# Ignaciagothe/tda-eeg-audio

Measured on AMD Instinct MI355X. Metric: windows/sec end-to-end (dist->Rips H0/H1->Wasserstein), 47-ch EEG, higher is better.
Workload: dtype f64; 1 GPU; configs[4]+configs[2]: 1416 recordings x 5 bands x 15 selected windows = 106200 (EEG 47x250 f64, audio 250 f64) window pairs per pass, the whole job; per pair corr->dist->Rips H0/H1 (EEG 47 pts), tau per recording-band, Takens dim 3 sub 2 + Rips (audio, 23..123 pts over the bands), Wasserstein H0+H1, features, per-recording reductions; one all-gather of the (1416, 5x48) rows per pass; windows_per_pass=106200, windows_per_gpu_per_pass=106200, input_bytes_per_gpu=10195200000, batches_per_pass=1, windows_per_batch=106200, parallelism=recordings dealt over 1 rank(s), one all-gather per pass, batches_in_flight=3, hip_graph=True, batches_rerun_with_full_ladder=0

## Files before the change

### tda_eeg_audio_amd/csrc/rips.hip

```cpp
#include "common.h"
#include "corr_dist_dev.h"
#include <stdlib.h>

#ifndef CLOUD_NB
#define CLOUD_NB 8192
#endif
#ifndef NARROW_NT
#define NARROW_NT 512
#endif
#ifndef NARROW_WAVES
#define NARROW_WAVES 6
#endif
#if defined(TDA_PROFILE) && !defined(TDA_PROFILE_STOPS_ONLY)
#define NARROW_NB (NARROW_NT == 384 ? 1536 : 1024)
#else
#define NARROW_NB (NARROW_NT == 384 ? 1536 : 2048)
#endif
#define NARROW_EMAX 7626
#define NT_MAX 512
#define RANK_NONE 0x7fffu

#ifdef TDA_PROFILE
__device__ unsigned long long g_prof[48];
#ifdef TDA_PROFILE_STOPS_ONLY
// ... 16 lines not shown
        prof_t0 = prof_t1;                                                 \
    } while (0)
#define PROF_COUNT(i, v) do { if (threadIdx.x == 0) prof_lds[i] += (unsigned long long)(v); } while (0)
#define PROF_FLUSH()                                                       \
    do {                                                                   \
        __syncthreads();                                                   \
        if (threadIdx.x < 48 && prof_lds[threadIdx.x]) atomicAdd(&g_prof[threadIdx.x], prof_lds[threadIdx.x]); \
    } while (0)
#endif
__device__ int g_stop_after;
extern "C" __attribute__((visibility("default"))) int tda_profile_stop_after(int n)
{
    return hipMemcpyToSymbol(HIP_SYMBOL(g_stop_after), &n, sizeof(int)) != hipSuccess;
}
#define PROF_STOP(n, cleanup) do { if (g_stop_after == (n)) { cleanup; return; } } while (0)
#define PROF_STOPC(n, cleanup) do { if (g_stop_after == (n) + 100 * prof_chunk) { cleanup; return; } } while (0)
extern "C" __attribute__((visibility("default"))) int tda_profile_read(unsigned long long* out, int reset)
{
    if (hipMemcpyFromSymbol(out, HIP_SYMBOL(g_prof), sizeof(unsigned long long) * 48) != hipSuccess) return 1;
    if (reset) {
        unsigned long long z[48] = {0};
        if (hipMemcpyToSymbol(HIP_SYMBOL(g_prof), z, sizeof(z)) != hipSuccess) return 1;
    }
    return 0;
}
#else
#define PROF_BEGIN() do {} while (0)
#define PROF_RESUME() do {} while (0)
#define PROF_MARK(i) do {} while (0)
#define PROF_COUNT(i, v) do {} while (0)
#define PROF_FLUSH() do {} while (0)
#define PROF_STOP(n, cleanup) do {} while (0)
#define PROF_STOPC(n, cleanup) do {} while (0)
#endif

#define LDS_ORDER() asm volatile("" ::: "memory")

#define LAUNDER(v) asm volatile("" : "+v"(v))
#define WAVE_SYNC()                                            \
    do {                                                       \
        __builtin_amdgcn_fence(__ATOMIC_ACQ_REL, "workgroup"); \
        __builtin_amdgcn_wave_barrier();                       \
    } while (0)

struct SweepShared {
    u64 alive[8];
    int cov_min[2], status, spare, k1, nk, more;
};

typedef unsigned short pk_u16 __attribute__((ext_vector_type(2)));
typedef short pk_i16 __attribute__((ext_vector_type(2)));

template <int W, typename WT>
struct __attribute__((aligned(sizeof(WT)))) Psi {
    WT w[W];
};
template <int W, typename WT>
__device__ __forceinline__ Psi<W, WT> pxor(Psi<W, WT> a, Psi<W, WT> b)
{
    Psi<W, WT> r;
#pragma unroll
    for (int i = 0; i < W; ++i) r.w[i] = a.w[i] ^ b.w[i];
    return r;
}
template <int W, typename WT>
__device__ __forceinline__ bool pnz(Psi<W, WT> a)
{
    WT o = 0;
#pragma unroll
    for (int i = 0; i < W; ++i) o |= a.w[i];
    return o != 0;
}
template <int W, typename WT>
__device__ __forceinline__ Psi<W, WT> pzero()
{
    Psi<W, WT> r;
#pragma unroll
    for (int i = 0; i < W; ++i) r.w[i] = 0;
    return r;
}

__device__ __forceinline__ double wave_min_f64(double v)
{
#pragma unroll
    for (int off = 32; off > 0; off >>= 1) { const double o = __shfl_xor(v, off, 64); v = o < v ? o : v; }
    return v;
}
__device__ __forceinline__ double wave_max_f64(double v)
{
#pragma unroll
    for (int off = 32; off > 0; off >>= 1) { const double o = __shfl_xor(v, off, 64); v = o > v ? o : v; }
    return v;
}

__device__ __forceinline__ int tri2(int v) { return (v * (v - 1)) >> 1; }
__device__ __forceinline__ int pair_index(int x, int y) { return x > y ? tri2(x) + y : tri2(y) + x; }

__device__ __forceinline__ int edge_row(int e)
{
    const int a = (int)((1.0f + __builtin_amdgcn_sqrtf(1.0f + 8.0f * (float)e)) * 0.5f);
    const int t = tri2(a);
    return a + (t + a <= e ? 1 : 0) - (t > e ? 1 : 0);
}

#ifndef TDA_NO_EDGE_TABLE
struct EdgeTable {
    u16 v[8192 + 512];
    constexpr EdgeTable() : v()
    {
        int a = 1, b = 0;
        for (int e = 0; e < 8192 + 512; ++e) { v[e] = (u16)((a << 8) | b); if (++b == a) { ++a; b = 0; } }
    }
};
__device__ const EdgeTable g_edge_ab = EdgeTable();
__device__ __forceinline__ u32 edge_ab(int e) { return (u32)g_edge_ab.v[e]; }
#else
__device__ __forceinline__ u32 edge_ab(int e) { const int a = edge_row(e); return (u32)((a << 8) | (e - tri2(a))); }
#endif

struct WgVote {
    u32* slots;
    int parity;
};
template <int NT>
__device__ __forceinline__ bool wg_any(WgVote& v, bool p)
{
    static_assert(NT % 64 == 0 && NT <= 512, "slots are read as one or two 16-byte words; slots beyond NT / 64 hold zero");
    const bool w = __ballot(p) != 0ull;
    u32* s = v.slots + 8 * v.parity;
    if ((threadIdx.x & 63) == 0) s[threadIdx.x >> 6] = w ? 1u : 0u;
    __syncthreads();
    v.parity ^= 1;
    const uint4 x = *reinterpret_cast<const uint4*>(s);
    u32 r = x.x | x.y | x.z | x.w;
    if (NT > 256) { const uint4 y = *reinterpret_cast<const uint4*>(s + 4); r |= y.x | y.y | y.z | y.w; }
    return r != 0u;
}
template <int NT>
__device__ __forceinline__ bool wg_all(WgVote& v, bool p) { return !wg_any<NT>(v, !p); }

__device__ __forceinline__ int wave_incl_scan_i32(int v)
{
#define TDA_DPP_ADD_(CTRL, RM) v += __builtin_amdgcn_update_dpp(0, v, CTRL, RM, 0xF, true)
    TDA_DPP_ADD_(0x111, 0xF);
    TDA_DPP_ADD_(0x112, 0xF);
    TDA_DPP_ADD_(0x114, 0xF);
    TDA_DPP_ADD_(0x118, 0xF);
    TDA_DPP_ADD_(0x142, 0xA);
    TDA_DPP_ADD_(0x143, 0xC);
#undef TDA_DPP_ADD_
    return v;
}

__device__ __forceinline__ int edge_flat(u32 pk) { return tri2((int)(pk >> 8)) + (int)(pk & 255u); }

struct Bucketer {
    float dmin, scale, top;
    __device__ __forceinline__ int operator()(u32 key) const
    {
        const float x = fminf((sortable_f32(key) - dmin) * scale, top);
        const int b = (int)x;
        return b < 0 ? 0 : b;
    }
};

template <int NT>
__device__ __forceinline__ void effective_threshold(int n, u32 tkey, const u32* vmax, u32 kmin_thread, u32* red, u32& teff_out, u32& kmin_out)
{
    const int tid = threadIdx.x;
    const int lane = tid & 63;
    const u32 m0 = lane < n ? vmax[lane] : 0xffffffffu, m1 = lane + 64 < n ? vmax[lane + 64] : 0xffffffffu;
    const u32 renc = wave_min_u32_dpp(m0 < m1 ? m0 : m1);
    teff_out = renc < tkey ? renc : tkey;
    if (tid == 0) red[1] = 0xffffffffu;
    __syncthreads();
    const u32 kmin = wave_min_u32_dpp(kmin_thread);
    if (lane == 63) atomicMin(&red[1], kmin);
    __syncthreads();
    kmin_out = red[1];
}

template <int NT, int NB, bool WANT_KEYS>
__device__ __forceinline__ int rank_edges(const u32* key32, int E, u32 teff, u32 kmin, u16* members, u32* cursor, int* wsum, u16* rank,
                          u16* ord, u32* skey)
{
    static_assert(NB % (2 * NT) == 0, "every thread scans whole words");
    constexpr int WPT = NB / NT / 2;
    const int tid = threadIdx.x, lane = tid & 63, wave = tid >> 6;
    Bucketer bk;
    bk.dmin = sortable_f32(kmin);
    bk.top = (float)(NB - 1);
    bk.scale = bk.top / (sortable_f32(teff) - bk.dmin);
    for (int i = tid; i < NB / 2; i += NT) cursor[i] = 0u;
    __syncthreads();
#pragma unroll 4
    for (int e = tid; e < E; e += NT) {
        const u32 k = key32[e];
        u32 b = 0xffffu;
        if (k <= teff) { b = (u32)bk(k); atomicAdd(&cursor[b >> 1], 1u << (16 * (b & 1))); }
        rank[e] = (u16)b;
    }
    __syncthreads();
    {
        u32 w[WPT];
        int s = 0;
#pragma unroll
        for (int i = 0; i < WPT; ++i) {
            const u32 x = cursor[tid * WPT + i];
            const int c0 = (int)(x & 0xffffu), c1 = (int)(x >> 16);
            w[i] = (u32)s | ((u32)(s + c0) << 16);
            s += c0 + c1;
        }
        const int incl = wave_incl_scan_i32(s);
        if (lane == 63) wsum[wave] = incl;
        __syncthreads();
        int basep = incl - s;
        for (int q = 0; q < wave; ++q) basep += wsum[q];
        const u32 add = (u32)basep * 0x00010001u;
#pragma unroll
        for (int i = 0; i < WPT; ++i) cursor[tid * WPT + i] = w[i] + add;
    }
    __syncthreads();
#pragma unroll 4
    for (int e = tid; e < E; e += NT) {
        const u32 b = rank[e];
        if (b != 0xffffu) {
            const int sh = 16 * (int)(b & 1u);
            const u32 old = atomicAdd(&cursor[b >> 1], 1u << sh);
            members[(old >> sh) & 0xffffu] = (u16)e;
        }
    }
    __syncthreads();
    const u16* cur16 = reinterpret_cast<const u16*>(cursor);
    const int Ev = uni((int)cur16[NB - 1]);
#pragma unroll 4
    for (int e = tid; e < E; e += NT) {
        const u32 b = rank[e];
        u32 r = RANK_NONE;
        if (b != 0xffffu) {
            const u32 k = key32[e];
            const int lo = b ? (int)cur16[b - 1] : 0, hi = (int)cur16[b];
            int c = 0;
            for (int j = lo; j < hi; ++j) {
                const u32 m = members[j];
                const u32 km = key32[m];
                c += (km < k || (km == k && m < (u32)e)) ? 1 : 0;
            }
            r = (u32)(lo + c);
        }
        rank[e] = (u16)r;
    }
    __syncthreads();
#pragma unroll 4
    for (int e = tid; e < E; e += NT) {
        const u32 r = rank[e];
        if (r != RANK_NONE) {
            ord[r] = (u16)edge_ab(e);
            if (WANT_KEYS) skey[r] = key32[e];
        }
    }
    __syncthreads();
    return Ev;
}

#if defined(TDA_PROFILE) && !defined(TDA_PROFILE_STOPS_ONLY)
#define NARROW_LDS ((160 * 1024 / 3 / 1280) * 1280 - 384)
#else
#define NARROW_LDS ((160 * 1024 / 3 / 1280) * 1280)
#endif
#define NARROW_PMAX 124
#define NARROW_DIM 3
#ifdef TDA_DEBUG_PTS
#define NL_GUARD 16
#else
#define NL_GUARD 0
#endif
#define NL_A16(x) (((x) + 15) & ~15)
struct NL {
    static constexpr int E = NARROW_EMAX;
    static constexpr int RANK = 0;
    static constexpr int PSI = NL_A16(2 * E) + NL_GUARD;
    static constexpr int MEMBERS = NL_A16(4 * E);
    static constexpr int CURSOR = NL_A16(MEMBERS + 2 * E);
    static constexpr int RSCR = CURSOR + 2 * NARROW_NB;
    static constexpr int TOTAL = NARROW_LDS;
    static constexpr int AUX = TOTAL - NL_GUARD - NL_A16(NARROW_PMAX * NARROW_DIM * 8);
    static constexpr int MISC = AUX - NL_GUARD - NL_A16(8752 + 8 * 32);
    static constexpr int REGION = MISC - NL_GUARD - PSI;
    static_assert(RSCR + 720 <= AUX - NL_GUARD, "the ranking arrays must end in front of the points");
    static_assert(MEMBERS >= 4 * (E + 1) && CURSOR >= MEMBERS + 2 * (E + 3), "room for the walk's padding (rank_edges_narrow)");
    static_assert(REGION >= 2 * E + 8 * 512, "the first chunks must fit: class vectors of 2 NT ranks next to the whole of ord");
};

template <int NT, int NB>
__device__ __forceinline__ int rank_edges_narrow(const u32* key32, int E, u32 teff, u32 kmin, u16* members, u32* cursor, int* wsum,
                                                 u16* rank, u16* ord)
{
    static_assert(NB % (2 * NT) == 0, "every thread scans whole words");
    static_assert(NB <= 0x8000, "bucket indices are parked in 16 bits, 0xffff = beyond the threshold");
    constexpr int WPT = NB / NT / 2;
    constexpr int EPT = 2 * ((NARROW_EMAX + 2 * NT - 1) / (2 * NT));
    const int tid = threadIdx.x, lane = tid & 63, wave = tid >> 6;
    Bucketer bk;
    bk.dmin = sortable_f32(kmin);
    bk.top = (float)(NB - 1);
    bk.scale = bk.top / (sortable_f32(teff) - bk.dmin);
// ... 23 lines not shown
        }
        const int incl = wave_incl_scan_i32(s);
        if (lane == 63) wsum[wave] = incl;
        __syncthreads();
        int basep = incl - s;
        for (int q = 0; q < wave; ++q) basep += wsum[q];
        const u32 add = (u32)basep * 0x00010001u;
#pragma unroll
        for (int i = 0; i < WPT; ++i) cursor[tid * WPT + i] = w[i] + add;
        if (tid == NT - 1) {
            const int total = basep + s;
            members[total] = (u16)NARROW_EMAX; members[total + 1] = (u16)NARROW_EMAX; members[total + 2] = (u16)NARROW_EMAX;
            const_cast<u32*>(key32)[NARROW_EMAX] = 0xffffffffu;
        }
    }
    __syncthreads();
#pragma unroll
    for (int i = 0; i < EPT; ++i) {
        const u32 b = i & 1 ? rk[i >> 1] >> 16 : rk[i >> 1] & 0xffffu;
        if (b != 0xffffu) {
            const int sh = 16 * (int)(b & 1u);
            const u32 old = atomicAdd(&cursor[b >> 1], 1u << sh);
            members[(old >> sh) & 0xffffu] = (u16)(tid + i * NT);
        }
    }
    __syncthreads();
    const u16* cur16 = reinterpret_cast<const u16*>(cursor);
    const int Ev = uni((int)cur16[NB - 1]);
#pragma unroll
    for (int i = 0; i < EPT; ++i) {
        const u32 e = (u32)(tid + i * NT);
        const u32 b = i & 1 ? rk[i >> 1] >> 16 : rk[i >> 1] & 0xffffu;
        u32 r = RANK_NONE;
        if (b != 0xffffu) {
            const u32 k = key32[e];
            const u64 me = ((u64)k << 32) | e;
            const int lo = b ? (int)cur16[b - 1] : 0, hi = (int)cur16[b];
            int c = 0;
            for (int j = lo; j < hi; j += 4) {
                u32 m[4], km[4];
#pragma unroll
                for (int t = 0; t < 4; ++t) m[t] = (u32)members[j + t];
#pragma unroll
                for (int t = 0; t < 4; ++t) km[t] = key32[m[t]];
#pragma unroll
                for (int t = 0; t < 4; ++t) c += ((((u64)km[t] << 32) | m[t]) < me) ? 1 : 0;
            }
            r = (u32)(lo + c);
        }
        if (i & 1) rk[i >> 1] = (rk[i >> 1] & 0xffffu) | (r << 16); else rk[i >> 1] = (rk[i >> 1] & 0xffff0000u) | r;
    }
    __syncthreads();
#pragma unroll
    for (int i = 0; i < EPT; ++i) {
        const int e = tid + i * NT;
        if (e < E) {
            const u32 r = i & 1 ? rk[i >> 1] >> 16 : rk[i >> 1] & 0xffffu;
            rank[e] = (u16)r;
            if (r != RANK_NONE) ord[r] = (u16)edge_ab(e);
        }
    }
    __syncthreads();
    return Ev;
}

struct RipsOut {
    double* h0; int h0_cap; int* h0_cnt;
    double* h1; int h1_cap; int* h1_cnt;
    int* status;
    int* retry_list = nullptr;
};

struct RipsLayout {
    int off_members;
    int off_rank, off_ord, off_aux, off_misc;
    int total;
    int off_psi, psi_bytes, off_cursor, off_rscr;
    int guard[5], n_guard;
};

#define TDA_WIN_LDS_GUARD 0x100
#ifndef TDA_SOLO_PRIO
#define TDA_SOLO_PRIO 3
#endif
#define TDA_SOLO_BEGIN() __builtin_amdgcn_s_setprio(TDA_SOLO_PRIO)
#define TDA_SOLO_END() __builtin_amdgcn_s_setprio(0)

#define TDA_POLL_LIMIT (1 << 16)
#ifndef TDA_TURN_SLEEP
#define TDA_TURN_SLEEP 4
#endif
#ifdef TDA_DEBUG_PTS
__device__ int g_fault;
extern "C" __attribute__((visibility("default"))) int tda_debug_inject(int what)
{
    return hipMemcpyToSymbol(HIP_SYMBOL(g_fault), &what, sizeof(int)) != hipSuccess;
}
#define TDA_FAULT(n) (g_fault == (n))
#else
#define TDA_FAULT(n) false
#endif
#ifdef TDA_DEBUG_PTS
#define GUARD_BYTES 16
__device__ __forceinline__ void guard_write(unsigned char* smem, const RipsLayout& L)
{
    if ((int)threadIdx.x < 4 * L.n_guard) reinterpret_cast<u32*>(smem + L.guard[threadIdx.x >> 2] - GUARD_BYTES)[threadIdx.x & 3] = 0xC0FFEE00u + threadIdx.x;
    __syncthreads();
}
__device__ __forceinline__ int guard_check(unsigned char* smem, const RipsLayout& L)
{
    __syncthreads();
    bool bad = false;
    if ((int)threadIdx.x < 4 * L.n_guard) bad = reinterpret_cast<u32*>(smem + L.guard[threadIdx.x >> 2] - GUARD_BYTES)[threadIdx.x & 3] != 0xC0FFEE00u + threadIdx.x;
    return __syncthreads_or(bad ? 1 : 0) ? TDA_WIN_LDS_GUARD : 0;
}
#else
#define GUARD_BYTES 0
__device__ __forceinline__ void guard_write(unsigned char*, const RipsLayout&) {}
__device__ __forceinline__ int guard_check(unsigned char*, const RipsLayout&) { return 0; }
#endif

#define MISC_COMP 0
#define MISC_CAND 512
#define MISC_WV (512 + 128)
#define MISC_MIN (512 + 192)
#define MISC_DONE (512 + 208)
#define MISC_SORTCNT (512 + 224)
#define MISC_SHARED (MISC_DONE + NT_MAX)
#define MISC_CKEY (MISC_SHARED + 96)
#define MISC_LIST MISC_CKEY
#define MISC_LIST_BYTES (4 * NT_MAX + 1280)
#define MISC_ADJ (MISC_LIST + MISC_LIST_BYTES)
#define MISC_ADJC (MISC_ADJ + 128 * 16)
#define MISC_BRANK (MISC_ADJC + 128 * 16)
#define MISC_BYTES(ncls) (MISC_BRANK + 8 * (ncls))

template <int NT, int NVW, int W, typename WT, bool NARROW, class KEYFN>
__device__ __forceinline__ void rips_sweep(int n, int E, int Ev, const u16* rank, const u16* ord, Psi<W, WT>* psi, int psi_bytes,
                           unsigned char* misc, KEYFN keyfn, double* h0, int h0_cap, double* h1, int h1_cap,
                           int& out_k0, int& out_k1, int& out_status)
{
    static_assert(!NARROW || W == 1, "the narrow layout is the point-cloud first pass");
    int psi_cap = 0;
    const int tid0 = threadIdx.x;
    const int lane0 = tid0 & 63, wave = uni(tid0 >> 6);
    int* brank = reinterpret_cast<int*>(misc + MISC_BRANK);
    u64* cand = reinterpret_cast<u64*>(misc + MISC_CAND);
    unsigned char* done = misc + MISC_DONE;
    SweepShared* shared = reinterpret_cast<SweepShared*>(misc + MISC_SHARED);
    u64* adj = reinterpret_cast<u64*>(misc + MISC_ADJ);
    constexpr int WB = 8 * (int)sizeof(WT);
    float* bkey = reinterpret_cast<float*>(misc + MISC_BRANK + 4 * WB * W);
    u64* adjc = reinterpret_cast<u64*>(misc + MISC_ADJC);

    if constexpr (!NARROW) for (int e = tid0; e < E; e += NT) psi[e] = pzero<W, WT>();
    for (int i = tid0; i < WB * W; i += NT) { brank[i] = -1; bkey[i] = 0.f; }
    for (int i = tid0; i < 256; i += NT) { adj[i] = 0ull; adjc[i] = 0ull; }
    if (tid0 == 0) {
        u32* lc = reinterpret_cast<u32*>(misc + MISC_MIN);
        lc[0] = 0u; lc[1] = 0xffffffffu; lc[2] = 0u;
        lc[3] = 0u;
        shared->status = 0;
    }
    if (tid0 < 16) {
        reinterpret_cast<u32*>(misc + MISC_WV)[tid0] = 0u;
        cand[tid0] = 0ull;
    }
    __syncthreads();

    WgVote vote{reinterpret_cast<u32*>(misc + MISC_WV), 0};
    WT alive[W];
#pragma unroll
    for (int c = 0; c < W; ++c) alive[c] = 0;
    int k0 = 0, k1 = 0, merges = 0, status = 0;
    int compA = lane0, compB = lane0 + 64;

    int clen = NT;
    int ordcls = 0;
    int cov_next = tid0;
#ifdef TDA_PROFILE
    int prof_rneed = 0, prof_chunk = -1;
#endif
    PROF_RESUME();
    for (int r0 = 0; r0 < Ev && !status; r0 += clen) {
        int tid = tid0;
        LAUNDER(tid);
        const int lane = tid & 63;
        clen = NT;
        PROF_MARK(15);
#ifdef TDA_PROFILE
        ++prof_chunk;
#endif
        PROF_COUNT(23, 1);
        const int r = r0 + tid;
        const bool valid = r < Ev;
        int a = 1, b = 0;
        if (valid) { const u32 pk = ord[r]; a = (int)(pk >> 8); b = (int)(pk & 255u); }
        const int tab = tri2(a) + b;
        const int slot = NARROW ? r : tab;
        if constexpr (NARROW) {
            psi_cap = (psi_bytes - 2 * (E - r0)) >> 2;
            if (r < psi_cap) psi[r] = pzero<W, WT>();
        }
        u64 M[NVW], M0[NVW];
        u64 Aj[NVW], Bj[NVW];
#pragma unroll
        for (int w = 0; w < NVW; ++w) { M[w] = 0; M0[w] = 0; Aj[w] = 0; Bj[w] = 0; }
        if (valid) {
#pragma unroll
            for (int w = 0; w < NVW; ++w) { Aj[w] = adj[2 * a + w]; Bj[w] = adj[2 * b + w]; M0[w] = Aj[w] & Bj[w]; }
        }
        {
            volatile u32* turn = reinterpret_cast<volatile u32*>(misc + MISC_MIN) + 2;
            if (wave > 0) {
                int trips = 0;
                for (;;) {
                    const u32 t = (u32)uni((int)*turn);
                    if (t >= (u32)wave) break;
                    if (++trips > TDA_POLL_LIMIT) { if (lane == 0) turn[1] = 1u; break; }
                    if (t + 1u < (u32)wave) __builtin_amdgcn_s_sleep(TDA_TURN_SLEEP); else __builtin_amdgcn_s_sleep(0);
                }
            }
            __builtin_amdgcn_fence(__ATOMIC_ACQUIRE, "workgroup");
            if (valid) {
#pragma unroll
                for (int w = 0; w < NVW; ++w) M[w] = (Aj[w] | adjc[2 * a + w]) & (Bj[w] | adjc[2 * b + w]);
                atomicOr(reinterpret_cast<unsigned long long*>(&adjc[2 * a + (b >> 6)]), 1ull << (b & 63));
                atomicOr(reinterpret_cast<unsigned long long*>(&adjc[2 * b + (a >> 6)]), 1ull << (a & 63));
            }
            LDS_ORDER();
            if (lane == 0 && !(TDA_FAULT(1) && wave == 3)) *turn = (u32)wave + 1u;
        }
        if (valid) {
            const int ta0 = tri2(a), tb0 = tri2(b);
#pragma unroll
            for (int w = 0; w < NVW; ++w) {
                u64 cc = (Aj[w] | adjc[2 * a + w]) & (Bj[w] | adjc[2 * b + w]) & ~M[w];
                while (cc) {
                    const int v0 = 64 * w + __builtin_ctzll(cc); cc &= cc - 1ull;
                    const bool ok1 = cc != 0ull; const int v1 = ok1 ? 64 * w + __builtin_ctzll(cc) : v0; cc &= cc - 1ull;
                    const int t0 = tri2(v0), t1 = tri2(v1);
                    const u32 xa0 = rank[v0 < a ? ta0 + v0 : t0 + a], xb0 = rank[v0 < b ? tb0 + v0 : t0 + b];
                    const u32 xa1 = rank[v1 < a ? ta0 + v1 : t1 + a], xb1 = rank[v1 < b ? tb0 + v1 : t1 + b];
                    if ((int)(xa0 > xb0 ? xa0 : xb0) < r) M[w] |= 1ull << (v0 & 63);
                    if (ok1 && (int)(xa1 > xb1 ? xa1 : xb1) < r) M[w] |= 1ull << (v1 & 63);
                }
            }
        }
        u64 many = 0;
#pragma unroll
        for (int w = 0; w < NVW; ++w) many |= M[w];
        const bool is_cand = valid && many == 0;
        int vstar = 0, d1 = 0, d2 = 0, q1 = 0, q2 = 0;
        {
            u64 many0 = 0;
#pragma unroll
            for (int w = 0; w < NVW; ++w) many0 |= M0[w];
            if (many0) {
                if (NVW == 1 || M0[0]) vstar = __builtin_ctzll(M0[0]);
                else vstar = 64 + __builtin_ctzll(M0[NVW - 1]);
            } else if (many) {
                if (NVW == 1 || M[0]) vstar = __builtin_ctzll(M[0]);
                else vstar = 64 + __builtin_ctzll(M[NVW - 1]);
            }
            if (valid && many != 0) {
                d1 = pair_index(a, vstar); d2 = pair_index(b, vstar);
                q1 = (int)rank[d1] - r0; q2 = (int)rank[d2] - r0;
                if (TDA_FAULT(2) && tid == 77 && q1 >= 0) q1 = tid;
            }
        }
        PROF_MARK(4);
        PROF_STOPC(11, out_k0 = k0; out_k1 = k1; out_status = 0);
        u64* mbal = reinterpret_cast<u64*>(misc + MISC_COMP);
        u64* zbal = mbal + 8;
        int* offs = reinterpret_cast<int*>(mbal + 16);
        u16* freebits = reinterpret_cast<u16*>(misc + MISC_CKEY);
        float mykey = 0.f;
        if (is_cand) mykey = keyfn(r, a, b);
        {
            const u64 bal = __ballot(is_cand), zb = __ballot(is_cand && mykey == 0.0f);
            if (lane == 0) { cand[wave] = bal; zbal[wave] = zb; }
        }
        done[tid] = 0;
        __syncthreads();
        PROF_MARK(21);
        PROF_STOPC(12, out_k0 = k0; out_k1 = k1; out_status = 0);
        int nfree = 0;
#pragma unroll
        for (int c = 0; c < W; ++c) nfree += __builtin_popcountll((u64)(WT)~alive[c]);
        int ncand = 0;
#pragma unroll
        for (int w = 0; w < NT / 64; ++w) ncand += __builtin_popcountll(cand[w]);
        int btot = 0;
        if (ncand > 0) {
        const bool par = ncand > 24;
        const int lblA0 = compA, lblB0 = compB;
        int qpar = NT;
        if (par) {
            int* bcomp = reinterpret_cast<int*>(misc + MISC_LIST + 1024);
            u32* bbest2 = reinterpret_cast<u32*>(bcomp + 128);
            int* bpar = reinterpret_cast<int*>(bcomp + 384);
            auto rounds = [&](int limit) {
                if (wave == 0) { bcomp[lane] = lblA0; bcomp[64 + lane] = lblB0; }
                if (tid < 256) bbest2[tid] = 0xffffffffu;
                __syncthreads();
                bool live = is_cand && tid < limit, picked = false;
                for (int round = 0; round < 64; ++round) {
                    u32* bbest = bbest2 + 128 * (round & 1);
                    int ca = 0, cb2 = 0;
                    if (live) {
                        ca = bcomp[a]; cb2 = bcomp[b];
                        if (ca == cb2) live = false;
                        else { atomicMin(&bbest[ca], (u32)tid); atomicMin(&bbest[cb2], (u32)tid); }
                    }
                    if (!wg_any<NT>(vote, live)) break;
                    if (live && (bbest[ca] == (u32)tid || bbest[cb2] == (u32)tid)) { picked = true; live = false; }
                    if (wave == 0) {
                        TDA_SOLO_BEGIN();
                        int pp[2];
#pragma unroll
                        for (int h = 0; h < 2; ++h) {
                            const int me = lane + 64 * h;
                            pp[h] = me;
                            const u32 bp = bbest[me];
                            if (bp != 0xffffffffu) {
                                const u32 pk = ord[r0 + (int)bp];
                                const int oa = bcomp[pk >> 8], ob = bcomp[pk & 255u];
                                pp[h] = oa == me ? ob : oa;
                                if (bbest[pp[h]] == bp && me < pp[h]) pp[h] = me;
                            }
                        }
                        bpar[lane] = pp[0]; bpar[64 + lane] = pp[1];
                        for (int it = 0; it < 8; ++it) {
                            const int p0 = bpar[lane], p1 = bpar[64 + lane];
                            const int g0 = bpar[p0], g1 = bpar[p1];
                            if (__ballot(g0 != p0 || g1 != p1) == 0ull) break;
                            bpar[lane] = g0; bpar[64 + lane] = g1;
                        }
                        const int c0 = bcomp[lane], c1 = bcomp[64 + lane];
                        const int n0 = bpar[c0], n1 = bpar[c1];
                        bcomp[lane] = n0; bcomp[64 + lane] = n1;
                        u32* other = bbest2 + 128 * ((round + 1) & 1);
                        other[lane] = 0xffffffffu; other[64 + lane] = 0xffffffffu;
                        TDA_SOLO_END();
                    }
                    __syncthreads();
                }
                const u64 mb = __ballot(picked);
                if (lane == 0) mbal[wave] = mb;
                __syncthreads();
            };
            rounds(NT);
            int nbirth = 0, wcut = -1, before = 0;
#pragma unroll
            for (int w = 0; w < NT / 64; ++w) {
                const int nb = __builtin_popcountll(cand[w] & ~mbal[w]);
                if (wcut < 0 && nbirth + nb > nfree) { wcut = w; before = nbirth; }
                nbirth += nb;
            }
            if (wcut >= 0) {
                u64 bw = cand[wcut] & ~mbal[wcut];
                for (int k = before; k < nfree; ++k) bw &= bw - 1ull;
                qpar = 64 * wcut + __builtin_ctzll(bw);
                PROF_COUNT(26, 1);
                __syncthreads();
                rounds(qpar);
            }
            if (wave == 0) { compA = bcomp[lane]; compB = bcomp[64 + lane]; }
        }
        if (wave == 0) {
            TDA_SOLO_BEGIN();
            const u64 candv = cand[lane & 7];
            int q = par ? qpar : NT, births = 0;
            const bool walk = !par;
            for (int g = 0; g < NT / 64 && walk; ++g) {
                u64 cb = q == NT ? rl64(candv, g) : 0ull;
                u64 mm = 0ull;
                if (cb) {
                    PROF_COUNT(20, __builtin_popcountll(cb));
                    const u32 pkv = ord[r0 + 64 * g + lane < E ? r0 + 64 * g + lane : E - 1];
                    while (cb) {
                        const int l = __builtin_ctzll(cb);
                        cb &= cb - 1;
                        const u32 pk = rl32(pkv, l);
                        const int qa = (int)(pk >> 8), qb = (int)(pk & 255u);
                        int ca, cbb;
                        if (NVW == 1) {
                            ca = (int)rl32((u32)compA, qa);
                            cbb = (int)rl32((u32)compA, qb);
                        } else {
                            const int a0 = (int)rl32((u32)compA, qa & 63), a1 = (int)rl32((u32)compB, qa & 63);
                            const int b0 = (int)rl32((u32)compA, qb & 63), b1 = (int)rl32((u32)compB, qb & 63);
                            ca = qa < 64 ? a0 : a1;
                            cbb = qb < 64 ? b0 : b1;
                        }
                        const bool same = ca == cbb, open = q == NT;
                        q = (open && same && births == nfree) ? 64 * g + l : q;
                        births += same ? 1 : 0;
                        const int cnew = (q == NT) ? ca : cbb;
                        compA = compA == cbb ? cnew : compA;
                        if (NVW == 2) compB = compB == cbb ? cnew : compB;
                        mm |= (!same && q == NT) ? (1ull << l) : 0ull;
                    }
                }
                if (lane == 0) mbal[g] = mm;
            }
            int nb = 0, nr = 0, nm = 0;
            if (lane < NT / 64) {
                u64 cg = cand[lane];
                if (64 * lane >= q) cg = 0ull;
                else if (q < 64 * lane + 64) cg &= (1ull << (q - 64 * lane)) - 1ull;
                const u64 mg = mbal[lane], zg = zbal[lane];
                nb = __builtin_popcountll(cg & ~mg); nr = __builtin_popcountll(mg & ~zg); nm = __builtin_popcountll(mg);
            }
            int pb = 0, pr = 0, tb = 0, tr = 0, tm = 0;
#pragma unroll
            for (int w = 0; w < NT / 64; ++w) {
                const int xb = (int)rl32((u32)nb, w), xr = (int)rl32((u32)nr, w), xm = (int)rl32((u32)nm, w);
                if (w < lane) { pb += xb; pr += xr; }
                tb += xb; tr += xr; tm += xm;
            }
            if (lane < NT / 64) { offs[lane] = pb; offs[8 + lane] = pr; }
            if (lane == 0) { offs[16] = tb; offs[17] = tr; offs[18] = tm; offs[19] = q; }
            TDA_SOLO_END();
        } else {
            for (int t = tid - 64; t < WB * W; t += NT - 64) {
                const int cw = t / WB, bit = t & (WB - 1);
                int rk = 0;
                bool fr = false;
#pragma unroll
                for (int c = 0; c < W; ++c) {
                    const WT f_ = (WT)~alive[c];
                    if (c < cw) rk += __builtin_popcountll((u64)f_);
                    if (c == cw) { rk += __builtin_popcountll((u64)(f_ & (((WT)1 << bit) - (WT)1))); fr = (f_ >> bit) & (WT)1; }
                }
                if (fr) freebits[rk] = (u16)t;
// ... 17 lines not shown
            if (row) {
                const int pos = k0 + rpre;
                if (pos < h0_cap) { h0[2 * pos] = 0.0; h0[2 * pos + 1] = (double)mykey; }
            }
            k0 += rtot; merges += mtot;
            if (birth) {
                const int idx = (int)freebits[bpre];
                const int cw = idx / WB, bit = idx & (WB - 1);
                Psi<W, WT> nv = pzero<W, WT>();
#pragma unroll
                for (int c = 0; c < W; ++c)
                    if (c == cw) nv.w[c] = ((WT)1 << bit);
                if (!NARROW || r < psi_cap) psi[slot] = nv;
                brank[idx] = r;
                bkey[idx] = mykey;
            }
            if (W == 1 && wave == 0 && btot > 0) {
                const int nal = __builtin_popcountll((u64)alive[0]);
                if (lane >= nal && lane < nal + btot) ordcls = (int)freebits[lane - nal];
            }
            int left = btot;
#pragma unroll
            for (int c = 0; c < W; ++c) {
                const u64 f_ = (u64)(WT)~alive[c];
                const int pc = __builtin_popcountll(f_);
                if (left >= pc) { alive[c] = (WT)~(WT)0; left -= pc; }
                else if (left > 0) {
                    int lo = 0, hi = 63;
                    while (lo < hi) {
                        const int mid = (lo + hi) >> 1;
                        if (__builtin_popcountll(f_ & ((2ull << mid) - 1ull)) >= left) hi = mid; else lo = mid + 1;
                    }
                    alive[c] |= (WT)(f_ & ((2ull << lo) - 1ull));
                    left = 0;
                }
            }
        }
        }
        if (status) break;
        PROF_MARK(5);
        PROF_STOPC(14, out_k0 = k0; out_k1 = k1; out_status = 0);
        bool quiet = btot == 0;
#pragma unroll
        for (int c = 0; c < W; ++c) quiet = quiet && alive[c] == 0;
        u32* lcnt = reinterpret_cast<u32*>(misc + MISC_MIN);
        if (quiet) PROF_COUNT(24, 1);
#ifdef TDA_PROFILE
        if (!quiet) prof_rneed = r0 + clen;
#endif
        if constexpr (NARROW) {
            if (!quiet && r0 + NT > psi_cap) { status |= TDA_WIN_CLASS_OVERFLOW; break; }
        }
        if (!quiet) {
        const bool apparent = valid && many != 0 && tid < clen;
        bool pending = apparent;
        Psi<W, WT> base = pzero<W, WT>();
        const int s1 = NARROW ? q1 + r0 : d1, s2 = NARROW ? q2 + r0 : d2;
        if (apparent && q1 < 0 && q2 < 0) {
            base = pxor(psi[s1], psi[s2]);
            psi[slot] = base;
            pending = false;
        }
        volatile unsigned char* vdone = done;
        LDS_ORDER();
        if (!pending) vdone[tid] = 1;
#ifdef TDA_PROFILE
#ifndef TDA_PROFILE_STOPS_ONLY
        if (pending) atomicAdd(&prof_lds[33], 1ull);
#endif
        PROF_COUNT(34, 1);
#endif
        int idle_trips = 0;
        while (__ballot(pending)) {
            PROF_COUNT(32, 1);
            bool ready = false;
            if (pending) ready = (q1 < 0 || vdone[q1]) && (q2 < 0 || vdone[q2]);
            const u64 rbal = __ballot(ready);
            __builtin_amdgcn_fence(__ATOMIC_ACQUIRE, "workgroup");
            if (ready) {
                base = pxor(psi[s1], psi[s2]);
                psi[slot] = base;
                LDS_ORDER();
                vdone[tid] = 1;
                pending = false;
            }
            if (!rbal) {
                if (++idle_trips > TDA_POLL_LIMIT) {
                    if (lane == 0) reinterpret_cast<volatile u32*>(misc + MISC_MIN)[3] = 1u;
                    if (pending) vdone[tid] = 1;
                    break;
                }
                __builtin_amdgcn_s_sleep(1);
            }
        }
        __syncthreads();
        PROF_MARK(6);
        PROF_STOPC(15, out_k0 = k0; out_k1 = k1; out_status = 0);
        u32 m0, m1, m2 = 0u, m3 = 0u;
        {
            u64 rem[NVW];
#pragma unroll
            for (int w = 0; w < NVW; ++w) rem[w] = 0ull;
            if (apparent) {
                u64 comp[NVW];
#pragma unroll
                for (int w = 0; w < NVW; ++w) comp[w] = 0ull;
                if (NVW == 1 || vstar < 64) comp[0] = 1ull << vstar;
                else comp[NVW - 1] = 1ull << (vstar - 64);
#pragma unroll
                for (int w = 0; w < NVW; ++w) { comp[w] |= adj[2 * vstar + w] & M[w]; rem[w] = M[w] & ~comp[w]; }
                bool changed = true;
                while (changed) {
                    changed = false;
#pragma unroll
                    for (int w = 0; w < NVW; ++w) {
                        u64 rr = rem[w];
                        while (rr) {
                            int u[4]; bool ok[4];
#pragma unroll
                            for (int k = 0; k < 4; ++k) {
                                ok[k] = rr != 0ull;
                                u[k] = ok[k] ? 64 * w + __builtin_ctzll(rr) : vstar;
                                rr &= rr - 1ull;
                            }
                            u64 nb[4][NVW];
#pragma unroll
                            for (int k = 0; k < 4; ++k)
#pragma unroll
                                for (int x = 0; x < NVW; ++x) nb[k][x] = adj[2 * u[k] + x];
#pragma unroll
                            for (int k = 0; k < 4; ++k) {
                                u64 hit = 0ull;
#pragma unroll
                                for (int x = 0; x < NVW; ++x) hit |= nb[k][x] & comp[x];
                                if (ok[k] && hit) {
                                    comp[w] |= 1ull << (u[k] & 63);
                                    rem[w] &= ~(1ull << (u[k] & 63));
                                    changed = true;
                                }
                            }
                        }
                    }
                    u64 anyr = 0ull;
#pragma unroll
                    for (int w = 0; w < NVW; ++w) anyr |= rem[w];
                    if (!anyr) break;
                }
            }
            m0 = (u32)rem[0]; m1 = (u32)(rem[0] >> 32);
            if (NVW == 2) { m2 = (u32)rem[NVW - 1]; m3 = (u32)(rem[NVW - 1] >> 32); }
        }
        PROF_MARK(16);
        PROF_STOPC(16, out_k0 = k0; out_k1 = k1; out_status = 0);
        const int ta_ = tri2(a), tb_ = tri2(b);
        constexpr int ES = 4 + W * (int)sizeof(WT);
        constexpr bool SORTED = W == 1;
        constexpr int HISTN = (NT + 255) & ~255;
        constexpr int HIST_BYTES = SORTED ? HISTN + 8 : 0;
        constexpr int LMAX = SORTED ? 255 : 256;
        constexpr int LCAP = ((MISC_LIST_BYTES - HIST_BYTES) / ES) < LMAX ? ((MISC_LIST_BYTES - HIST_BYTES) / ES) : LMAX;
        constexpr int LPL = (LCAP + 63) / 64;
        constexpr bool FTAB = WB * W * (int)sizeof(Psi<W, WT>) <= MISC_LIST_BYTES;
        constexpr int KMAX = FTAB ? 64 : LCAP;
        unsigned char* list = misc + MISC_LIST;
        unsigned char* hist = list + ((LCAP * ES + 7) & ~7);
        const u32 mws[4] = {m0, m1, m2, m3};
#ifdef TDA_PROFILE
        {
            const int ntri = __builtin_popcount(m0) + __builtin_popcount(m1) + __builtin_popcount(m2) + __builtin_popcount(m3);
#ifndef TDA_PROFILE_STOPS_ONLY
            if (ntri) atomicAdd(&prof_lds[27], (unsigned long long)ntri);
            if (apparent) atomicAdd(&prof_lds[28], 1ull);
            if (ntri) atomicAdd(&prof_lds[29], 1ull);
#endif
        }
#endif
        int list_rounds = 0;
        while (true) {
            if (list_rounds > 0) {
                if (tid == 0) { lcnt[0] = 0u; lcnt[1] = 0xffffffffu; }
                __syncthreads();
            }
            u32 firstkey = 0xffffffffu;
            Psi<W, WT> firsty = pzero<W, WT>();
            u32 mycnt = 0u;
            if (apparent) {
                base = psi[slot];
                Psi<W, WT> prev = pzero<W, WT>();
#pragma unroll
                for (int wi = 0; wi < NVW; ++wi) {
                    u64 mm = (u64)mws[2 * wi] | ((u64)mws[2 * wi + 1] << 32);
                    const int vbase = 64 * wi;
                    while (mm) {
                        const int v0 = vbase + __builtin_ctzll(mm); mm &= mm - 1ull;
                        const bool ok1 = mm != 0ull; const int v1 = ok1 ? vbase + __builtin_ctzll(mm) : v0; mm &= mm - 1ull;
                        const bool ok2 = mm != 0ull; const int v2 = ok2 ? vbase + __builtin_ctzll(mm) : v0; mm &= mm - 1ull;
                        const bool ok3 = mm != 0ull; const int v3 = ok3 ? vbase + __builtin_ctzll(mm) : v0; mm &= mm - 1ull;
#define TDA_IDX_(v, ja, jb)                                                       \
                        const int t##ja = (int)(__umul24((u32)(v), (u32)((v) - 1)) >> 1); \
                        const int f##ja = (v) < a ? ta_ + (v) : t##ja + a;                 \
                        const int f##jb = (v) < b ? tb_ + (v) : t##ja + b;                 \
                        const int ja = NARROW ? (int)rank[f##ja] : f##ja;                  \
                        const int jb = NARROW ? (int)rank[f##jb] : f##jb;
                        TDA_IDX_(v0, ja0, jb0) TDA_IDX_(v1, ja1, jb1) TDA_IDX_(v2, ja2, jb2) TDA_IDX_(v3, ja3, jb3)
#undef TDA_IDX_
                        const Psi<W, WT> p0 = psi[ja0], q0 = psi[jb0], p1 = psi[ja1], q1_ = psi[jb1];
                        const Psi<W, WT> p2 = psi[ja2], q2_ = psi[jb2], p3 = psi[ja3], q3 = psi[jb3];
                        const Psi<W, WT> ys[4] = {pxor(pxor(p0, q0), base), pxor(pxor(p1, q1_), base),
                                                  pxor(pxor(p2, q2_), base), pxor(pxor(p3, q3), base)};
                        const bool oks[4] = {true, ok1, ok2, ok3};
                        const int vs[4] = {v0, v1, v2, v3};
#pragma unroll
                        for (int k = 0; k < 4; ++k) {
                            if (!oks[k] || !pnz(ys[k]) || !pnz(pxor(ys[k], prev))) continue;
                            prev = ys[k];
                            const u32 key = ((u32)tid << 8) | (u32)vs[k];
                            if (firstkey == 0xffffffffu) { firstkey = key; firsty = ys[k]; }
                            const u32 idx = atomicAdd(&lcnt[0], 1u);
                            if (idx < (u32)LCAP) {
                                *reinterpret_cast<u32*>(list + ES * idx) = SORTED ? key | (mycnt << 24) : key;
#pragma unroll
                                for (int c = 0; c < W; ++c)
                                    *reinterpret_cast<WT*>(list + ES * idx + 4 + c * (int)sizeof(WT)) = ys[k].w[c];
                            }
                            ++mycnt;
                        }
                    }
                }
            }
            if (SORTED) {
                hist[tid] = (unsigned char)mycnt;
                if (NT < HISTN && tid < HISTN - NT) hist[NT + tid] = 0;
            }
            {
                const u32 wmin = wave_min_u32_dpp(firstkey);
                if (lane == 0 && wmin != 0xffffffffu) atomicMin(&lcnt[1], wmin);
            }
            __syncthreads();
            PROF_MARK(17);
            PROF_STOPC(17, out_k0 = k0; out_k1 = k1; out_status = 0);
            const u32 cnt = (u32)uni((int)lcnt[0]);
            if (cnt == 0u) break;
            const bool complete = cnt <= (u32)LCAP;
            PROF_COUNT(11, 1);
            PROF_COUNT(12, cnt);
            if (!complete) {
                PROF_COUNT(13, 1);
                if (firstkey == lcnt[1]) {
                    *reinterpret_cast<u32*>(list) = firstkey;
#pragma unroll
                    for (int c = 0; c < W; ++c) *reinterpret_cast<WT*>(list + 4 + c * (int)sizeof(WT)) = firsty.w[c];
                }
                __syncthreads();
            }
            WT alive_before[W];
#pragma unroll
            for (int c = 0; c < W; ++c) alive_before[c] = alive[c];
            if (wave == 0) {
                TDA_SOLO_BEGIN();
                const int nl = complete ? (int)cnt : 1;
                u32 ek[LPL];
                Psi<W, WT> ev[LPL];
#pragma unroll
                for (int q = 0; q < LPL; ++q) {
                    const int idx = lane + 64 * q;
                    ek[q] = 0xffffffffu; ev[q] = pzero<W, WT>();
                    if (idx < nl) {
                        ek[q] = *reinterpret_cast<const u32*>(list + ES * idx);
#pragma unroll
                        for (int c = 0; c < W; ++c)
                            ev[q].w[c] = *reinterpret_cast<const WT*>(list + ES * idx + 4 + c * (int)sizeof(WT));
                    }
                }
                if (SORTED && complete) {
                    constexpr int HW = HISTN / 256;
                    u32* hw = reinterpret_cast<u32*>(hist) + HW * lane;
                    const u32 x0 = hw[0], x1 = HW == 2 ? hw[HW - 1] : 0u;
                    const u32 s0 = __builtin_amdgcn_sad_u8(x0, 0u, 0u);
                    const u32 tot = HW == 2 ? __builtin_amdgcn_sad_u8(x1, 0u, s0) : s0;
                    const u32 before = (u32)wave_incl_scan_i32((int)tot) - tot;
                    hw[0] = x0 * 0x01010101u - x0 + before * 0x01010101u;
                    if (HW == 2) hw[HW - 1] = x1 * 0x01010101u - x1 + (before + s0) * 0x01010101u;
#pragma unroll
                    for (int q = 0; q < LPL; ++q) {
                        if (lane + 64 * q < nl) {
                            const int pos = (int)hist[(ek[q] >> 8) & 0xffffu] + (int)(ek[q] >> 24);
                            *reinterpret_cast<u32*>(list + ES * pos) = ek[q] & 0x00ffffffu;
                            *reinterpret_cast<WT*>(list + ES * pos + 4) = ev[q].w[0];
                        }
                    }
#pragma unroll
                    for (int q = 0; q < LPL; ++q) {
                        const int idx = lane + 64 * q;
                        if (idx < nl) {
                            ek[q] = *reinterpret_cast<const u32*>(list + ES * idx);
                            ev[q].w[0] = *reinterpret_cast<const WT*>(list + ES * idx + 4);
                        }
                    }
                }
                const int lb = lane & (WB - 1);
                int brk[W];
                float bky[W];
#pragma unroll
                for (int c = 0; c < W; ++c) {
                    brk[c] = lane < WB ? brank[WB * c + lb] : -1;
                    bky[c] = lane < WB ? bkey[WB * c + lb] : 0.f;
                }
                int nalive0 = W == 1 ? __builtin_popcountll((u64)alive[0]) : 0;
                Psi<W, WT> vimg = pzero<W, WT>();
                u32 mycode = 0u, myrk = 0u;
                float mybirth = 0.f;
                int nk = 0, more = 0;
                const int nq = (nl + 63) >> 6;
                PROF_MARK(30);
                if constexpr (SORTED) {
                    WT kvec = 0;
                    WT cm = lane < nalive0 ? (WT)1 << ordcls : (WT)0;
                    bool stop = false;
#pragma unroll
                    for (int q = 0; q < LPL; ++q) {
                        if (q >= nq || stop) break;
                        WT v = ev[q].w[0];
                        const u32 myk = ek[q];
                        for (int k = 0; k < nk; ++k) {
                            const WT m = (WT)1 << rl32(mycode, k);
                            const WT w = sizeof(WT) == 8 ? (WT)rl64((u64)kvec, k) : (WT)rl32((u32)kvec, k);
                            if (v & m) v ^= w;
                        }
                        u64 nz = __ballot(v != 0);
                        while (nz) {
                            if (nk == KMAX) { more = 1; stop = true; break; }
                            const int src = __builtin_ctzll(nz);
                            const WT wvw = sizeof(WT) == 8 ? (WT)rl64((u64)v, src) : (WT)rl32((u32)v, src);
                            const u64 ob = __ballot((cm & wvw) != 0);
                            if (!ob) { status |= TDA_WIN_CLASS_OVERFLOW; stop = true; break; }
                            const int opos = 63 - __builtin_clzll(ob);
                            const int ybit = (int)rl32((u32)ordcls, opos);
                            const WT ybm = (WT)1 << ybit;
                            if (v & ybm) v ^= wvw;
                            nz = __ballot(v != 0);
                            const u32 kk = rl32(myk, src);
                            const float ybirth = __uint_as_float(rl32(__float_as_uint(bky[0]), ybit));
                            cm &= (WT)~ybm;
                            const bool me = lane == nk;
                            WT vi = vimg.w[0];
                            if (vi & ybm) vi ^= wvw;
                            vimg.w[0] = me ? (WT)(wvw & (WT)~ybm) : vi;
                            mycode = me ? (u32)ybit : mycode;
                            myrk = me ? (u32)(r0 + (int)((kk >> 8) & 0xffffu)) : myrk;
                            mybirth = me ? ybirth : mybirth;
                            kvec = me ? wvw : kvec;
                            alive[0] &= (WT)~ybm;
                            ++nk;
                        }
                    }
                    if (nk > 0) {
                        const bool keep = cm != 0;
                        const u64 keepb = __ballot(keep);
                        const int below = (int)__builtin_amdgcn_mbcnt_hi((u32)(keepb >> 32), __builtin_amdgcn_mbcnt_lo((u32)keepb, 0u));
                        const int dst = keep ? below : __builtin_popcountll(keepb) + (lane - below);
                        ordcls = __builtin_amdgcn_ds_permute(dst << 2, ordcls);
                    }
                } else
                while (true) {
                    u32 mk = 0xffffffffu;
#pragma unroll
                    for (int q = 0; q < LPL; ++q)
                        if (q < nq && pnz(ev[q]) && ek[q] < mk) mk = ek[q];
                    const u32 best = wave_min_u32_dpp(mk);
                    if (best == 0xffffffffu) break;
                    if (nk == KMAX) { more = 1; break; }
                    const int src = __builtin_ctzll(__ballot(mk == best));
                    Psi<W, WT> mine = pzero<W, WT>();
#pragma unroll
                    for (int q = 0; q < LPL; ++q)
                        if (q < nq && ek[q] == best) mine = ev[q];
                    Psi<W, WT> wv;
#pragma unroll
                    for (int c = 0; c < W; ++c) {
                        if (sizeof(WT) == 8) wv.w[c] = (WT)rl64((u64)mine.w[c], src);
                        else wv.w[c] = (WT)rl32((u32)mine.w[c], src);
                    }
                    const int rk = r0 + (int)(best >> 8);
                    int ybit, ycw;
                    float ybirth;
                    if (W == 1) {
                        const u64 ob = __ballot(lane < nalive0 && (((u64)wv.w[0] >> ordcls) & 1ull));
                        if (!ob) { status |= TDA_WIN_CLASS_OVERFLOW; break; }
                        const int opos = 63 - __builtin_clzll(ob);
                        ybit = (int)rl32((u32)ordcls, opos);
                        ycw = 0;
                        ybirth = __uint_as_float(rl32(__float_as_uint(bky[0]), ybit));
                        const int up = __builtin_amdgcn_update_dpp(0, ordcls, 0x130, 0xF, 0xF, true);
                        if (lane >= opos) ordcls = up;
                        --nalive0;
                    } else {
                        int candv = -1, cwl = 0;
                        float byl = 0.f;
#pragma unroll
                        for (int c = 0; c < W; ++c)
                            if (lane < WB && ((wv.w[c] >> lb) & (WT)1) && brk[c] > candv) { candv = brk[c]; cwl = c; byl = bky[c]; }
                        const int bestr = wave_max_i32_dpp(candv);
                        const u64 ybal = __ballot(candv == bestr && candv >= 0);
                        if (!ybal) { status |= TDA_WIN_CLASS_OVERFLOW; break; }
                        ybit = __builtin_ctzll(ybal);
                        ycw = (int)rl32((u32)cwl, ybit);
                        ybirth = __uint_as_float(rl32(__float_as_uint(byl), ybit));
                    }
                    if (FTAB) {
                        WT sel = 0;
#pragma unroll
                        for (int c = 0; c < W; ++c)
                            if (c == ycw) sel = (vimg.w[c] >> ybit) & (WT)1;
                        if (lane < nk && sel) vimg = pxor(vimg, wv);
                        if (lane == nk) {
                            vimg = wv;
#pragma unroll
                            for (int c = 0; c < W; ++c)
                                if (c == ycw) vimg.w[c] &= (WT)~((WT)1 << ybit);
                            mycode = ((u32)ycw << 8) | (u32)ybit; myrk = (u32)rk; mybirth = ybirth;
                        }
                    } else {
                        const u32 pkk = ord[rk];
                        const float key = keyfn(rk, (int)(pkk >> 8), (int)(pkk & 255u));
                        if (key > ybirth) {
                            if (k1 < h1_cap && lane == 0) { h1[2 * k1] = (double)ybirth; h1[2 * k1 + 1] = (double)key; }
                            ++k1;
                        }
                        if (lane == 0) {
                            *reinterpret_cast<u32*>(list + ES * nk) = ((u32)ycw << 8) | (u32)ybit;
#pragma unroll
                            for (int c = 0; c < W; ++c) *reinterpret_cast<WT*>(list + ES * nk + 4 + c * (int)sizeof(WT)) = wv.w[c];
                        }
                    }
#pragma unroll
                    for (int q = 0; q < LPL; ++q) {
                        if (q >= nq) break;
                        WT sel = 0;
#pragma unroll
                        for (int c = 0; c < W; ++c)
                            if (c == ycw) sel = (ev[q].w[c] >> ybit) & (WT)1;
                        if (sel) ev[q] = pxor(ev[q], wv);
                    }
#pragma unroll
                    for (int c = 0; c < W; ++c)
                        if (c == ycw) alive[c] &= (WT)~((WT)1 << ybit);
                    ++nk;
                }
                PROF_MARK(31);
                PROF_COUNT(10, nk);
// ... 1214 lines not shown
```

Before: 4.492 million windows/s.

## Distribute triangle list building across threads with scanned work lists

```diff
diff --git a/tda_eeg_audio_amd/csrc/rips.hip b/tda_eeg_audio_amd/csrc/rips.hip
--- a/tda_eeg_audio_amd/csrc/rips.hip
+++ b/tda_eeg_audio_amd/csrc/rips.hip
@@ -192,6 +192,42 @@
     return v;
 }
 
+__device__ __forceinline__ u32 wave_shr1_u32(u32 v) { return (u32)__builtin_amdgcn_update_dpp(0, (int)v, 0x138, 0xF, 0xF, true); }
+
+template <int W, typename WT>
+__device__ __forceinline__ Psi<W, WT> last_nonzero_of_owner(Psi<W, WT> y, u32 own1)
+{
+    constexpr int H = (int)sizeof(WT) / 4;
+    u32 x[W * H];
+    {
+        const bool mine = wave_shr1_u32(own1) == own1;
+#pragma unroll
+        for (int i = 0; i < W * H; ++i) {
+            const u32 below = wave_shr1_u32((u32)((u64)y.w[i / H] >> (32 * (i % H))));
+            x[i] = mine ? below : 0u;
+        }
+    }
+#define TDA_STEP_(CTRL)                                                                                              \
+    {                                                                                                                \
+        u32 any = 0u;                                                                                                \
+        _Pragma("unroll") for (int i = 0; i < W * H; ++i) any |= x[i];                                               \
+        const bool take = any == 0u && (u32)__builtin_amdgcn_update_dpp(0, (int)own1, CTRL, 0xF, 0xF, true) == own1; \
+        _Pragma("unroll") for (int i = 0; i < W * H; ++i) {                                                          \
+            const u32 o = (u32)__builtin_amdgcn_update_dpp(0, (int)x[i], CTRL, 0xF, 0xF, true);                      \
+            x[i] = take ? o : x[i];                                                                                  \
+        }                                                                                                            \
+    }
+    TDA_STEP_(0x111) TDA_STEP_(0x112) TDA_STEP_(0x114)
+#undef TDA_STEP_
+    Psi<W, WT> r;
+#pragma unroll
+    for (int c = 0; c < W; ++c) {
+        if constexpr (H == 2) r.w[c] = (WT)(((u64)x[2 * c + 1] << 32) | x[2 * c]);
+        else r.w[c] = (WT)x[c];
+    }
+    return r;
+}
+
 __device__ __forceinline__ int edge_flat(u32 pk) { return tri2((int)(pk >> 8)) + (int)(pk & 255u); }
 
 struct Bucketer {
@@ -521,6 +557,9 @@
     constexpr int WB = 8 * (int)sizeof(WT);
     float* bkey = reinterpret_cast<float*>(misc + MISC_BRANK + 4 * WB * W);
     u64* adjc = reinterpret_cast<u64*>(misc + MISC_ADJC);
+    int* tcum = reinterpret_cast<int*>(misc + MISC_COMP + 256);
+    int* ecum = reinterpret_cast<int*>(misc + MISC_COMP + 320);
+    int eset = 0;
 
     if constexpr (!NARROW) for (int e = tid0; e < E; e += NT) psi[e] = pzero<W, WT>();
     for (int i = tid0; i < WB * W; i += NT) { brank[i] = -1; bkey[i] = 0.f; }
@@ -651,6 +690,7 @@
             if (lane == 0) { cand[wave] = bal; zbal[wave] = zb; }
         }
         done[tid] = 0;
+        if (tid < 9) tcum[tid] = 0;
         __syncthreads();
         PROF_MARK(21);
         PROF_STOPC(12, out_k0 = k0; out_k1 = k1; out_status = 0);
@@ -974,7 +1014,6 @@
         }
         PROF_MARK(16);
         PROF_STOPC(16, out_k0 = k0; out_k1 = k1; out_status = 0);
-        const int ta_ = tri2(a), tb_ = tri2(b);
         constexpr int ES = 4 + W * (int)sizeof(WT);
         constexpr bool SORTED = W == 1;
         constexpr int HISTN = (NT + 255) & ~255;
@@ -985,8 +1024,19 @@
         constexpr bool FTAB = WB * W * (int)sizeof(Psi<W, WT>) <= MISC_LIST_BYTES;
         constexpr int KMAX = FTAB ? 64 : LCAP;
         unsigned char* list = misc + MISC_LIST;
-        unsigned char* hist = list + ((LCAP * ES + 7) & ~7);
-        const u32 mws[4] = {m0, m1, m2, m3};
+        u32* tlist = reinterpret_cast<u32*>(adjc);
+        static_assert(4 * NT <= 128 * 16 && NT / 64 <= 8, "the work list lives in adjc; nine words per sum");
+        const bool cum_lane = lane == 8 || (lane < 8 && lane > wave);
+        const int ntri = __builtin_popcount(m0) + __builtin_popcount(m1) + __builtin_popcount(m2) + __builtin_popcount(m3);
+        int tstart, ttot;
+        const int incl_ = wave_incl_scan_i32(ntri);
+        const int wtri = __builtin_amdgcn_readlane(incl_, 63);
+        {
+            if (wtri != 0 && cum_lane) atomicAdd(&tcum[lane], wtri);
+            __syncthreads();
+            tstart = tcum[wave] + incl_ - ntri;
+            ttot = uni(tcum[8]);
+        }
 #ifdef TDA_PROFILE
         {
             const int ntri = __builtin_popcount(m0) + __builtin_popcount(m1) + __builtin_popcount(m2) + __builtin_popcount(m3);
@@ -999,82 +1049,80 @@
 #endif
         int list_rounds = 0;
         while (true) {
-            if (list_rounds > 0) {
-                if (tid == 0) { lcnt[0] = 0u; lcnt[1] = 0xffffffffu; }
+            u64 left[NVW];
+            left[0] = (u64)m0 | ((u64)m1 << 32);
+            if (NVW == 2) left[NVW - 1] = (u64)m2 | ((u64)m3 << 32);
+            int nxt = tstart;
+            int lbase = 0;
+#ifdef TDA_PROFILE
+            {
+                PROF_COUNT(43, (ttot + NT - 1) / NT); PROF_COUNT(44, ttot); PROF_COUNT(47, 1);
+#ifndef TDA_PROFILE_STOPS_ONLY
+                if (wtri != 0 && lane == 0) atomicAdd(&prof_lds[45], 1ull);
+#endif
+            }
+#endif
+            for (int t0 = 0; t0 < ttot; t0 += NT) {
+                int* ec = ecum + 16 * eset;
+                eset ^= 1;
+                if (tid < 9) ec[tid] = 0;
+#pragma unroll
+                for (int wi = 0; wi < NVW; ++wi) {
+                    while (left[wi] != 0ull && (u32)(nxt - t0) < (u32)NT) {
+                        const int v = 64 * wi + __builtin_ctzll(left[wi]);
+                        left[wi] &= left[wi] - 1ull;
+                        tlist[nxt - t0] = ((u32)tid << 8) | (u32)v;
+                        ++nxt;
+                    }
+                }
                 __syncthreads();
-            }
-            u32 firstkey = 0xffffffffu;
-            Psi<W, WT> firsty = pzero<W, WT>();
-            u32 mycnt = 0u;
-            if (apparent) {
-                base = psi[slot];
-                Psi<W, WT> prev = pzero<W, WT>();
-#pragma unroll
-                for (int wi = 0; wi < NVW; ++wi) {
-                    u64 mm = (u64)mws[2 * wi] | ((u64)mws[2 * wi + 1] << 32);
-                    const int vbase = 64 * wi;
-                    while (mm) {
-                        const int v0 = vbase + __builtin_ctzll(mm); mm &= mm - 1ull;
-                        const bool ok1 = mm != 0ull; const int v1 = ok1 ? vbase + __builtin_ctzll(mm) : v0; mm &= mm - 1ull;
-                        const bool ok2 = mm != 0ull; const int v2 = ok2 ? vbase + __builtin_ctzll(mm) : v0; mm &= mm - 1ull;
-                        const bool ok3 = mm != 0ull; const int v3 = ok3 ? vbase + __builtin_ctzll(mm) : v0; mm &= mm - 1ull;
-#define TDA_IDX_(v, ja, jb)                                                       \
-                        const int t##ja = (int)(__umul24((u32)(v), (u32)((v) - 1)) >> 1); \
-                        const int f##ja = (v) < a ? ta_ + (v) : t##ja + a;                 \
-                        const int f##jb = (v) < b ? tb_ + (v) : t##ja + b;                 \
-                        const int ja = NARROW ? (int)rank[f##ja] : f##ja;                  \
-                        const int jb = NARROW ? (int)rank[f##jb] : f##jb;
-                        TDA_IDX_(v0, ja0, jb0) TDA_IDX_(v1, ja1, jb1) TDA_IDX_(v2, ja2, jb2) TDA_IDX_(v3, ja3, jb3)
-#undef TDA_IDX_
-                        const Psi<W, WT> p0 = psi[ja0], q0 = psi[jb0], p1 = psi[ja1], q1_ = psi[jb1];
-                        const Psi<W, WT> p2 = psi[ja2], q2_ = psi[jb2], p3 = psi[ja3], q3 = psi[jb3];
-                        const Psi<W, WT> ys[4] = {pxor(pxor(p0, q0), base), pxor(pxor(p1, q1_), base),
-                                                  pxor(pxor(p2, q2_), base), pxor(pxor(p3, q3), base)};
-                        const bool oks[4] = {true, ok1, ok2, ok3};
-                        const int vs[4] = {v0, v1, v2, v3};
-#pragma unroll
-                        for (int k = 0; k < 4; ++k) {
-                            if (!oks[k] || !pnz(ys[k]) || !pnz(pxor(ys[k], prev))) continue;
-                            prev = ys[k];
-                            const u32 key = ((u32)tid << 8) | (u32)vs[k];
-                            if (firstkey == 0xffffffffu) { firstkey = key; firsty = ys[k]; }
-                            const u32 idx = atomicAdd(&lcnt[0], 1u);
-                            if (idx < (u32)LCAP) {
-                                *reinterpret_cast<u32*>(list + ES * idx) = SORTED ? key | (mycnt << 24) : key;
-#pragma unroll
-                                for (int c = 0; c < W; ++c)
-                                    *reinterpret_cast<WT*>(list + ES * idx + 4 + c * (int)sizeof(WT)) = ys[k].w[c];
-                            }
-                            ++mycnt;
-                        }
+                u32 code = 0u;
+                Psi<W, WT> y = pzero<W, WT>();
+                bool keep = false;
+                u64 kb = 0ull;
+                if (t0 + (wave << 6) < ttot) {
+                    const bool item = t0 + tid < ttot;
+                    if (item) {
+                        code = tlist[tid];
+                        const int op = (int)(code >> 8), v = (int)(code & 255u);
+                        const u32 pk = ord[r0 + op];
+                        const int oa = (int)(pk >> 8), ob = (int)(pk & 255u);
+                        const int ta_ = tri2(oa), tb_ = tri2(ob);
+                        const int tv = (int)(__umul24((u32)v, (u32)(v - 1)) >> 1);
+                        const int fa = v < oa ? ta_ + v : tv + oa;
+                        const int fb = v < ob ? tb_ + v : tv + ob;
+                        const int ja = NARROW ? (int)rank[fa] : fa;
+                        const int jb = NARROW ? (int)rank[fb] : fb;
+                        y = pxor(pxor(psi[ja], psi[jb]), psi[NARROW ? r0 + op : ta_ + ob]);
                     }
-                }
-            }
-            if (SORTED) {
-                hist[tid] = (unsigned char)mycnt;
-                if (NT < HISTN && tid < HISTN - NT) hist[NT + tid] = 0;
-            }
-            {
-                const u32 wmin = wave_min_u32_dpp(firstkey);
-                if (lane == 0 && wmin != 0xffffffffu) atomicMin(&lcnt[1], wmin);
+                    const Psi<W, WT> pv = last_nonzero_of_owner(y, item ? (code >> 8) + 1u : 0u);
+                    keep = pnz(y) && pnz(pxor(y, pv));
+                    kb = __ballot(keep);
+                }
+                if (kb != 0ull && cum_lane) atomicAdd(&ec[lane], __builtin_popcountll(kb));
+                __syncthreads();
+                const int pos = lbase + ec[wave] + (int)__builtin_amdgcn_mbcnt_hi((u32)(kb >> 32), __builtin_amdgcn_mbcnt_lo((u32)kb, 0u));
+                lbase += uni(ec[8]);
+                if (keep && pos < LCAP) {
+                    *reinterpret_cast<u32*>(list + ES * pos) = code;
+#pragma unroll
+                    for (int c = 0; c < W; ++c)
+                        *reinterpret_cast<WT*>(list + ES * pos + 4 + c * (int)sizeof(WT)) = y.w[c];
+                }
+            }
+            if (lbase == 0) {
+                PROF_MARK(17);
+                PROF_STOPC(17, out_k0 = k0; out_k1 = k1; out_status = 0);
+                break;
             }
             __syncthreads();
             PROF_MARK(17);
             PROF_STOPC(17, out_k0 = k0; out_k1 = k1; out_status = 0);
-            const u32 cnt = (u32)uni((int)lcnt[0]);
-            if (cnt == 0u) break;
+            const u32 cnt = (u32)lbase;
             const bool complete = cnt <= (u32)LCAP;
             PROF_COUNT(11, 1);
             PROF_COUNT(12, cnt);
-            if (!complete) {
-                PROF_COUNT(13, 1);
-                if (firstkey == lcnt[1]) {
-                    *reinterpret_cast<u32*>(list) = firstkey;
-#pragma unroll
-                    for (int c = 0; c < W; ++c) *reinterpret_cast<WT*>(list + 4 + c * (int)sizeof(WT)) = firsty.w[c];
-                }
-                __syncthreads();
-            }
+            if (!complete) PROF_COUNT(13, 1);
             WT alive_before[W];
 #pragma unroll
             for (int c = 0; c < W; ++c) alive_before[c] = alive[c];
@@ -1092,32 +1140,6 @@
 #pragma unroll
                         for (int c = 0; c < W; ++c)
                             ev[q].w[c] = *reinterpret_cast<const WT*>(list + ES * idx + 4 + c * (int)sizeof(WT));
-                    }
-                }
-                if (SORTED && complete) {
-                    constexpr int HW = HISTN / 256;
-                    u32* hw = reinterpret_cast<u32*>(hist) + HW * lane;
-                    const u32 x0 = hw[0], x1 = HW == 2 ? hw[HW - 1] : 0u;
-                    const u32 s0 = __builtin_amdgcn_sad_u8(x0, 0u, 0u);
-                    const u32 tot = HW == 2 ? __builtin_amdgcn_sad_u8(x1, 0u, s0) : s0;
-                    const u32 before = (u32)wave_incl_scan_i32((int)tot) - tot;
-                    hw[0] = x0 * 0x01010101u - x0 + before * 0x01010101u;
-                    if (HW == 2) hw[HW - 1] = x1 * 0x01010101u - x1 + (before + s0) * 0x01010101u;
-#pragma unroll
-                    for (int q = 0; q < LPL; ++q) {
-                        if (lane + 64 * q < nl) {
-                            const int pos = (int)hist[(ek[q] >> 8) & 0xffffu] + (int)(ek[q] >> 24);
-                            *reinterpret_cast<u32*>(list + ES * pos) = ek[q] & 0x00ffffffu;
-                            *reinterpret_cast<WT*>(list + ES * pos + 4) = ev[q].w[0];
-                        }
-                    }
-#pragma unroll
-                    for (int q = 0; q < LPL; ++q) {
-                        const int idx = lane + 64 * q;
-                        if (idx < nl) {
-                            ek[q] = *reinterpret_cast<const u32*>(list + ES * idx);
-                            ev[q].w[0] = *reinterpret_cast<const WT*>(list + ES * idx + 4);
-                        }
                     }
                 }
                 const int lb = lane & (WB - 1);
```

After: 4.549 million windows/s (median of 6 runs). 1.01x the previous value.
